# EBI-Metagenomics/deciphon-old

Measured on AMD Instinct MI355X. Metric: Gcell-updates/sec, higher is better.
Workload: dtype f32

## Files before the change

### deciphon-old_amd/__init__.py

```python
import ctypes as C
import os
import subprocess

import numpy as np

_HERE = os.path.dirname(os.path.abspath(__file__))
ROOT = os.path.dirname(_HERE)
LIB_PATH = os.path.join(_HERE, "libdcp_hip.so")
CSRC = os.path.join(_HERE, "csrc")

RC_OK, RC_END, RC_EFAIL, RC_EINVAL, RC_EIO, RC_ENOMEM, RC_EPARSE, RC_EAPI, RC_EHTTP = range(9)
RC_NAMES = ["RC_OK", "RC_END", "RC_EFAIL", "RC_EINVAL", "RC_EIO", "RC_ENOMEM", "RC_EPARSE",
            "RC_EAPI", "RC_EHTTP"]
ENTRY_DIST_NULL, ENTRY_DIST_UNIFORM, ENTRY_DIST_OCCUPANCY = 0, 1, 2
NCODES = 1364
NDIST = 129
NXTRANS = 13
CORE_SIZE_MAX = 4096
NUM_THREADS = 64

ABI_SYMBOLS = [
    "dcp_profile_new", "dcp_profile_sample", "dcp_profile_del", "dcp_profile_core_size",
    "dcp_profile_from_parts", "dcp_profile_entry_dist", "dcp_profile_epsilon", "dcp_rnd_seed", "dcp_rnd_next",
    "dcp_dist_unique_id", "dcp_dist_init", "dcp_dist_init_from_file", "dcp_dist_free", "dcp_dist_rank",
# ... 2 lines not shown
    "dcp_dist_comm_count", "dcp_dist_last_gather_ms", "dcp_plan_query_slots",
    "dcp_lprob_normalize", "dcp_h3reader_open_fp", "dcp_h3reader_next_params", "dcp_gpu_seqs_set_xtrans",
    "dcp_profile_accession", "dcp_profile_trans8", "dcp_profile_null_dist",
    "dcp_profile_insert_dist", "dcp_profile_match_dist", "dcp_frame_table_host", "dcp_xtrans",
    "dcp_lrt", "dcp_partition_by_count", "dcp_partition_by_cells", "dcp_gpu_device_count",
    "dcp_gpu_ctx_new", "dcp_gpu_ctx_del", "dcp_gpu_last_error", "dcp_gpu_stream",
    "dcp_gpu_db_upload", "dcp_gpu_db_nprofiles", "dcp_gpu_db_fetch_match_table",
    "dcp_gpu_db_one_layout", "dcp_gpu_db_table_bytes",
    "dcp_gpu_seqs_upload", "dcp_gpu_seqs_upload_text", "dcp_gpu_nseqs", "dcp_gpu_scan",
    "dcp_gpu_sync", "dcp_gpu_last_scan_kernel", "dcp_gpu_hit_buffer", "dcp_gpu_last_scan_redo_pairs", "dcp_gpu_last_scan_ms", "dcp_gpu_last_scan_launches", "dcp_gpu_fetch_scores",
    "dcp_gpu_fetch_hits", "dcp_gpu_scan_range", "dcp_gpu_set_hit_buffer",
    "dcp_gpu_last_scan_launch_info", "dcp_gpu_scan_cells", "dcp_gpu_scan_algorithmic_bytes",
    "dcp_gpu_trace_paths", "dcp_state_name", "dcp_profile_decode", "dcp_gc_decode",
    "dcp_prod_format_row", "dcp_prod_header", "dcp_h3reader_open", "dcp_h3reader_next",
    "dcp_h3reader_error", "dcp_h3reader_close", "dcp_swissprot_null_lprobs", "dcp_profile_consensus",
    "dcp_db_write", "dcp_db_open", "dcp_db_close", "dcp_db_nprofiles", "dcp_db_entry_dist", "dcp_db_epsilon",
    "dcp_db_profile_sizes", "dcp_db_partitions", "dcp_db_read",
    "dcp_profile_new64", "dcp_profile_sample64", "dcp_profile_precision", "dcp_profile_epsilon64",
    "dcp_profile_trans8_64", "dcp_profile_null_dist64", "dcp_profile_insert_dist64", "dcp_profile_match_dist64",
    "dcp_xtrans64", "dcp_gpu_db_upload64", "dcp_gpu_db_precision", "dcp_gpu_set_lrt_threshold64", "dcp_gpu_fetch_scores64", "dcp_gpu_fetch_hits64",
    "dcp_gpu_db_fetch_match_table64", "dcp_gpu_db_fetch_insert_null64", "dcp_gpu_trace_paths64",
    "dcp_gpu_seqs_set_xtrans64", "dcp_profile_from_parts64", "dcp_lprob_normalize64",
    "dcp_gpu_last_scan_query_plan",
]


class DcpError(RuntimeError):
    def __init__(self, rc, msg=""):
        self.rc = rc
        name = RC_NAMES[rc] if 0 <= rc < len(RC_NAMES) else str(rc)
        super().__init__(f"{name}: {msg}" if msg else name)


def build(verbose=False):
    subprocess.check_call(["make", "-C", CSRC] + ([] if verbose else ["-s"]))
    return LIB_PATH


class ScanParams(C.Structure):
    _fields_ = [("multi_hits", C.c_int), ("hmmer3_compat", C.c_int),
                ("lrt_threshold", C.c_float), ("keep_scores", C.c_int), ("kernel", C.c_int)]


KERNEL_AUTO, KERNEL_ROWSWEEP, KERNEL_QLANE, KERNEL_QLANE2 = 0, 1, 2, 3
KERNEL_QLANE64 = 4
DB_EXPAND_ON_HOST, DB_ONE_LAYOUT = 1, 2
# ... 45 lines not shown
        "dcp_partition_by_count": (U, [U, U, P]),
        "dcp_partition_by_cells": (None, [P, U, U, P]),
        "dcp_gpu_device_count": (I, []),
        "dcp_gpu_ctx_new": (P, [I]),
        "dcp_gpu_ctx_del": (None, [P]),
        "dcp_gpu_last_error": (C.c_char_p, [P]),
        "dcp_gpu_stream": (P, [P]),
        "dcp_gpu_db_upload": (I, [P, P, U, I]),
        "dcp_gpu_db_nprofiles": (U, [P]),
        "dcp_gpu_db_one_layout": (I, [P]),
        "dcp_gpu_db_table_bytes": (C.c_uint64, [P]),
        "dcp_gpu_db_fetch_match_table": (I, [P, U, P]),
        "dcp_gpu_seqs_upload": (I, [P, P, P, U]),
        "dcp_gpu_seqs_upload_text": (I, [P, C.c_char_p, P, U]),
        "dcp_gpu_nseqs": (U, [P]),
        "dcp_gpu_seqs_set_xtrans": (I, [P, P, U]),
        "dcp_gpu_scan": (I, [P, C.POINTER(ScanParams)]),
        "dcp_gpu_sync": (I, [P]),
        "dcp_gpu_last_scan_redo_pairs": (I, [P, C.POINTER(U)]),
        "dcp_gpu_last_scan_query_plan": (I, [P, C.POINTER(U), C.POINTER(C.c_ulonglong), C.POINTER(U), C.POINTER(U)]),
        "dcp_gpu_last_scan_ms": (F, [P]),
        "dcp_gpu_last_scan_launches": (U, [P]),
        "dcp_gpu_last_scan_kernel": (I, [P]),
        "dcp_gpu_fetch_scores": (I, [P, P, P]),
        "dcp_gpu_fetch_hits": (I, [P, P, U, C.POINTER(U)]),
        "dcp_gpu_scan_range": (I, [P, C.POINTER(ScanParams), U, U]),
        "dcp_gpu_set_hit_buffer": (I, [P, P, U, P]),
        "dcp_gpu_last_scan_launch_info": (I, [P, U, C.POINTER(LaunchInfo)]),
        "dcp_gpu_trace_paths": (I, [P, P, U, I, I, I, P, U, P, P]),
        "dcp_state_name": (U, [U, C.c_char_p]),
        "dcp_profile_decode": (I, [P, P, U, U, P]),
        "dcp_gc_decode": (C.c_char, [P]),
        "dcp_prod_format_row": (C.c_long, [C.c_char_p, C.c_size_t, C.c_int64, C.c_int64, C.c_char_p, C.c_char_p,
                                           C.c_double, C.c_double, C.c_char_p, C.c_char_p, P, P, U, P, U]),
        "dcp_prod_header": (C.c_char_p, []),
        "dcp_h3reader_open": (P, [C.c_char_p, I, F]),
        "dcp_h3reader_next": (I, [P, C.POINTER(P)]),
        "dcp_h3reader_error": (C.c_char_p, [P]),
        "dcp_h3reader_close": (None, [P]),
        "dcp_swissprot_null_lprobs": (None, [P]),
        "dcp_profile_consensus": (C.c_char_p, [P]),
        "dcp_db_write": (I, [C.c_char_p, P, U]),
        "dcp_db_open": (P, [C.c_char_p, C.POINTER(I)]),
        "dcp_db_close": (None, [P]),
        "dcp_db_nprofiles": (U, [P]),
        "dcp_db_entry_dist": (I, [P]),
# ... 483 lines not shown
        self._check(self._lib.dcp_gpu_test_set_trace_mode(self._c, int(bool(own_forward)), int(budget_floats)))

    def test_table_span(self, p):
        span, ldk, eb = C.c_uint(0), C.c_uint(0), C.c_uint(0)
        self._check(self._lib.dcp_gpu_test_fetch_table_span(self._c, p, None, 0, C.byref(span), C.byref(ldk),
                                                            C.byref(eb)))
        out = np.zeros((NCODES, span.value), np.float64 if eb.value == 8 else np.float32)
        self._check(self._lib.dcp_gpu_test_fetch_table_span(self._c, p, out.ctypes.data, out.nbytes, C.byref(span),
                                                            C.byref(ldk), C.byref(eb)))
        return out, ldk.value

    def test_set_rowsweep_variant(self, stage_rows, block_waves=0):
        self._check(self._lib.dcp_gpu_test_set_rowsweep_variant(self._c, int(stage_rows), int(block_waves)))

    @property
    def last_scan_ms(self):
        return self._lib.dcp_gpu_last_scan_ms(self._c)

    @property
    def last_scan_kernel(self):
        return self._lib.dcp_gpu_last_scan_kernel(self._c)

    @property
    def last_scan_launches(self):
        return self._lib.dcp_gpu_last_scan_launches(self._c)

    @property
    def last_scan_query_plan(self):
        nb, rows, prow, mg = C.c_uint(0), C.c_ulonglong(0), C.c_uint(0), C.c_uint(0)
        self._check(self._lib.dcp_gpu_last_scan_query_plan(self._c, C.byref(nb), C.byref(rows), C.byref(prow),
                                                           C.byref(mg)))
        return dict(nblocks=nb.value, sum_block_rows=rows.value, plane_rows=prow.value,
                    max_groups_per_slot=mg.value)

    @property
    def last_scan_redo_pairs(self):
        n = C.c_uint(0)
        self._check(self._lib.dcp_gpu_last_scan_redo_pairs(self._c, C.byref(n)))
        return n.value

    @property
    def cells(self):
        return self._lib.dcp_gpu_scan_cells(self._c)

    @property
    def algorithmic_bytes(self):
# ... 41 lines not shown
```

### deciphon-old_amd/csrc/dcp_gpu.hip

```cpp
#include "dcp_kernels.h"
#include "dcp_f64.h"

#include <hip/hip_runtime.h>

#include <algorithm>
#include <cmath>
#include <cstdarg>
#include <cstdio>
#include <cstring>
#include <limits>
#include <map>
#include <new>
#include <numeric>
#include <string>
#include <queue>
#include <type_traits>
#include <vector>

namespace
{

struct SizeClass
{
    int R, W;
// ... 139 lines not shown
    DevBuf<uint32_t> d_slot_first;
    unsigned ql_nqb = 0, ql_plane_rows = 0;
    unsigned ring_stall = 0;
    bool ring_check_pending = false;
    uint32_t *h_qstage = nullptr;
    size_t h_qstage_n = 0;
    hipEvent_t ev_qstage = nullptr;
    int rs_force_stg = -1;
    unsigned rs_force_bw = 0;
    unsigned rs_pad_lds = 0;
    int rs_force_pf = 0;
    int rs_force_R = 0;
    bool any_exact_e = false;
    DevBuf<unsigned> d_task_counter;
    DevBuf<dcp_pair> d_redo;
    DevBuf<unsigned> d_redo_n;
    bool redo_pending = false;
    unsigned last_redo_pairs = 0;
    struct dcp_scan_params last_prm = {};
    unsigned qorder_q0 = ~0u, qorder_q1 = ~0u, qorder_lmax = 0;
    unsigned num_cus = 0;
    int last_kernel = 0;
    unsigned qorder_nt = 0;
    int last_kernel_variant = 0;
    unsigned redo_cap_limit = 1u << 26;
    float last_ql_ms = 0;

    unsigned nseqs = 0;
    uint64_t total_len = 0;
    std::vector<uint32_t> seq_len;
    DevBuf<uint32_t> d_seq_words, d_seq_woff, d_seq_len;
    DevBuf<float> d_xtrans;
    int xt_multi = -1, xt_h3 = -1;
    bool xt_explicit = false;
    std::vector<double> xt64;

    ScanResults<float, dcp_hit> res;
    unsigned last_launches = 0;
    bool scanned = false;
    unsigned last_q0 = 0, last_q1 = 0;
    static constexpr int kMaxLaunches = 2 * kNumClasses + 1;
    hipEvent_t ev_class[kMaxLaunches] = {nullptr};
    hipStream_t class_stream[kNumClasses] = {nullptr};
    hipEvent_t ev_trace[kNumClasses + 1] = {nullptr};
    bool last_overlapped = false;
    int launched_class[kMaxLaunches] = {0};
// ... 1128 lines not shown
}

int dcp_gpu_hit_buffer(dcp_gpu_ctx *c, void **hits_dev, void **nhits_dev, unsigned *cap)
{
    if (!c || !hits_dev || !nhits_dev || !cap) return DCP_EINVAL;
    if (!c->scanned) return c->fail(DCP_EINVAL, "no scan yet");
    if (c->last_f64) return c->fail(DCP_EINVAL, "the last scan ran on a double DB: its hits are struct dcp_hit64 (dcp_gpu_fetch_hits64)");
    *hits_dev = c->res.hits();
    *nhits_dev = c->res.nhits();
    *cap = c->res.cap();
    return DCP_OK;
}

struct QlPlan
{
    std::vector<dcp_ql_group> groups;
    std::vector<uint32_t> slot_first;
    std::vector<uint32_t> block_rows;
    unsigned nqb = 0;
    unsigned plane_rows = 0;
    uint64_t sum_block_rows = 0;
    unsigned busy_slots = 0;
};
static QlPlan plan_query_groups(unsigned const *len_sorted, unsigned nq, unsigned slots)
{
    QlPlan pl;
    unsigned const ng = (nq + 63u) / 64u;
    struct G
    {
        unsigned first, n, lmax, rows;
    };
    std::vector<G> gs(ng);
    uint64_t sum_rows = 0;
    unsigned max_rows = 0;
    unsigned const rem = nq % 64u;
    for (unsigned g = 0; g < ng; ++g)
    {
        unsigned const first = rem == 0u ? g * 64u : (g == 0u ? 0u : rem + (g - 1u) * 64u);
        unsigned const n = rem != 0u && g == 0u ? rem : 64u;
        unsigned const lmax = len_sorted[first + n - 1u];
        gs[g] = G{first, n, lmax, dcp_qlane_group_rows(lmax)};
        sum_rows += gs[g].rows;
        max_rows = std::max(max_rows, gs[g].rows);
    }
    auto pack = [&](unsigned nqb, std::vector<std::vector<unsigned>> &slot_groups, std::vector<uint64_t> &load) {
        unsigned const S = nqb * slots;
        slot_groups.assign(S, {});
// ... 6 lines not shown
        {
            LS top = heap.top();
            heap.pop();
            slot_groups[top.second].push_back(g);
            load[top.second] += gs[g].rows;
            heap.push(LS(load[top.second], top.second));
        }
        std::vector<unsigned> order(S);
        for (unsigned i = 0; i < S; ++i)
            order[i] = i;
        std::stable_sort(order.begin(), order.end(), [&](unsigned x, unsigned y) { return load[x] > load[y]; });
        std::vector<std::vector<unsigned>> sg(S);
        std::vector<uint64_t> ld(S);
        for (unsigned i = 0; i < S; ++i)
            sg[i] = std::move(slot_groups[order[i]]), ld[i] = load[order[i]];
        slot_groups.swap(sg), load.swap(ld);
        uint64_t cost = 0;
        for (unsigned b = 0; b < nqb; ++b)
            cost += load[(size_t)b * slots];
        return cost;
    };
    unsigned const cap = (ng + slots - 1u) / slots;
    uint64_t const denom = (uint64_t)slots * max_rows;
    unsigned const lo = (unsigned)std::min<uint64_t>(std::max<uint64_t>(sum_rows / denom, 1), cap);
    unsigned const hi = (unsigned)std::min<uint64_t>(std::max<uint64_t>((sum_rows + denom - 1u) / denom, 1), cap);
    std::vector<std::vector<unsigned>> best_sg, sg;
    std::vector<uint64_t> best_ld, ld;
    uint64_t best_cost = ~0ull;
    unsigned best_nqb = 0;
    for (unsigned nqb = lo; nqb <= hi; ++nqb)
    {
        uint64_t const cost = pack(nqb, sg, ld);
        if (cost <= best_cost) best_cost = cost, best_nqb = nqb, best_sg.swap(sg), best_ld.swap(ld);
    }
    pl.nqb = best_nqb;
    pl.sum_block_rows = best_cost;
    pl.slot_first.assign((size_t)best_nqb * slots + 1u, 0);
    pl.block_rows.assign(best_nqb, 0);
    for (unsigned sidx = 0; sidx < best_nqb * slots; ++sidx)
    {
        pl.slot_first[sidx] = (uint32_t)pl.groups.size();
        uint32_t rowbase = 0;
        for (unsigned g : best_sg[sidx])
        {
            pl.groups.push_back(dcp_ql_group{gs[g].first, gs[g].n, rowbase, gs[g].lmax});
            rowbase += gs[g].rows;
        }
        pl.block_rows[sidx / slots] = std::max<uint32_t>(pl.block_rows[sidx / slots], rowbase);
        if (sidx < slots && rowbase) ++pl.busy_slots;
    }
    pl.slot_first.back() = (uint32_t)pl.groups.size();
    for (unsigned b = 0; b < best_nqb; ++b)
        pl.plane_rows = std::max(pl.plane_rows, pl.block_rows[b]);
    return pl;
}

namespace
{
struct SortedQueries
{
    std::vector<uint32_t> order;
    std::vector<unsigned> len;
    QlPlan plan;
};
}
static SortedQueries sorted_query_plan(dcp_gpu_ctx const *c, unsigned q_begin, unsigned q_end, unsigned slots)
{
    unsigned const nq = q_end - q_begin;
    SortedQueries s;
    s.order.resize(nq);
    std::iota(s.order.begin(), s.order.end(), 0u);
    std::stable_sort(s.order.begin(), s.order.end(),
                     [&](uint32_t x, uint32_t y) { return c->seq_len[q_begin + x] < c->seq_len[q_begin + y]; });
    s.len.resize(nq);
    for (unsigned i = 0; i < nq; ++i)
        s.len[i] = c->seq_len[q_begin + s.order[i]];
    s.plan = plan_query_groups(s.len.data(), nq, slots);
    return s;
}

extern "C" int dcp_plan_query_slots(unsigned const *len_sorted, unsigned nq, unsigned slots_per_block, unsigned *nblocks,
                                    unsigned long long *sum_block_rows, unsigned *plane_rows, unsigned *groups4,
                                    unsigned group_cap, unsigned *slot_first, unsigned slot_cap)
{
    if (!len_sorted || nq == 0 || (slots_per_block != 1u && slots_per_block != 4u) || !nblocks) return DCP_EINVAL;
    for (unsigned i = 1; i < nq; ++i)
        if (len_sorted[i] < len_sorted[i - 1]) return DCP_EINVAL;
    QlPlan const pl = plan_query_groups(len_sorted, nq, slots_per_block);
    *nblocks = pl.nqb;
    if (sum_block_rows) *sum_block_rows = pl.sum_block_rows;
    if (plane_rows) *plane_rows = pl.plane_rows;
    if (groups4)
    {
        if (group_cap < pl.groups.size()) return DCP_ENOMEM;
        std::memcpy(groups4, pl.groups.data(), pl.groups.size() * sizeof(dcp_ql_group));
    }
    if (slot_first)
    {
        if (slot_cap < pl.slot_first.size()) return DCP_ENOMEM;
        std::memcpy(slot_first, pl.slot_first.data(), pl.slot_first.size() * sizeof(uint32_t));
    }
    return DCP_OK;
}

static void rowsweep_variant(dcp_gpu_ctx const *c, int R, int W, unsigned nchunks, int *stg, unsigned *bw, int *pf)
{
    *pf = 0;
    if (W != 1)
    {
        *stg = 0, *bw = 1;
        return;
    }
    auto balanced = [&](unsigned maxw) {
        unsigned const nb = (nchunks + maxw - 1u) / maxw;
        return (nchunks + nb - 1u) / nb;
    };
    int g = 20;
    unsigned w = balanced(nchunks <= 56u ? 8u : 4u);
    unsigned const max84 = dcp_rowsweep_max_block_waves(R, W, 84);
    if (nchunks >= 6u && nchunks <= 36u && max84 != 0u)
    {
        unsigned const w84 = balanced(max84);
        unsigned const slots = dcp_rowsweep_max_block_waves(R, W, 84);
        unsigned const blocks = (160u * 1024u) / dcp_rowsweep_stage_bytes(R, 84);
        if (std::min(blocks * w84, slots) * 2u >= slots) g = 84, w = w84;
// ... 222 lines not shown
    double sum_len = 0;
    for (unsigned L : sorted.len)
        sum_len += L;
    unsigned const nqb = plan.nqb;
    double const sum_block_lmax = (double)plan.sum_block_rows;
    unsigned const lmax = sorted.len.back();
    double t_rs = (double)c->sum_core * (DCP_NCODES * 4.0) / 3e12 + qchunk * lmax * 1.2e-6;
    for (int k = 0; k < kNumClasses; ++k)
        t_rs += 1.05 * (double)c->class_core[k] * sum_len / kClassRate[k];
    unsigned const waves = std::max(1u, std::min(4u, plan.busy_slots));
    static double const kTrow[4] = {0.52, 0.54, 0.62, 0.73};
    double const trow = (w3 ? 0.56 : kTrow[waves - 1u]) * 1e-6;
    double const resident = (double)std::min<uint64_t>((uint64_t)c->nprof * nqb, (uint64_t)ql_blocks_per_cu * c->num_cus);
    double const t_ql = std::max((double)c->max_tiles * lmax * 0.52e-6,
                                 (double)c->sum_tiles * sum_block_lmax * trow / resident) +
                        1e-4;
    bool const stage2 = nq > 192u;
    double const fill = std::min(1.0, (double)c->nprof * nqb / (4.0 * c->num_cus));
    double const t_q = stage2 ? t_ql * (0.66 + 0.28 * fill) : t_ql;
    if (lmax > 200000u) return 1;
    return t_q < t_rs ? (stage2 ? 3 : 2) : 1;
}

static int ensure_qlane_layout(dcp_gpu_ctx *c, dcp_scan_args const &a, unsigned q_begin, unsigned q_end, unsigned ql_nt)
{
    if (!c->d_task_counter.p) HIP_TRY(c, c->d_task_counter.alloc(1));
    if (c->qorder_q0 == q_begin && c->qorder_q1 == q_end && c->qorder_nt == ql_nt) return DCP_OK;
    unsigned const nq = q_end - q_begin, NTq = ql_nt, slots = NTq / 64u;
    SortedQueries const sorted = sorted_query_plan(c, q_begin, q_end, slots);
    QlPlan const &plan = sorted.plan;
    unsigned const nqb = plan.nqb;
    if ((uint64_t)plan.plane_rows * NTq * 4u > 0xffffffffull)
        return c->fail(DCP_ENOMEM, "sequences too long for the query-lane kernel (%u plane rows): use kernel = 1", plan.plane_rows);
    size_t const nslot_words = (size_t)nqb * slots + 1u, ngroup_words = plan.groups.size() * 4u;
    size_t const need_stage = (size_t)nq + nqb + 1u + nslot_words + ngroup_words;
    if (!c->ev_qstage) HIP_TRY(c, hipEventCreateWithFlags(&c->ev_qstage, hipEventDisableTiming));
    else HIP_TRY(c, hipEventSynchronize(c->ev_qstage));
    if (c->h_qstage_n < need_stage)
    {
        if (c->h_qstage) (void)hipHostFree(c->h_qstage);
        c->h_qstage = nullptr, c->h_qstage_n = 0;
        HIP_TRY(c, hipHostMalloc((void **)&c->h_qstage, need_stage * sizeof(uint32_t), hipHostMallocDefault));
        c->h_qstage_n = need_stage;
    }
    uint32_t *const h_ord = c->h_qstage, *const wt_off = h_ord + nq, *const h_slots = wt_off + nqb + 1u,
                   *const h_groups = h_slots + nslot_words;
    static_assert(sizeof(dcp_ql_group) == 4 * sizeof(uint32_t), "group records travel as four words");
    std::memcpy(h_ord, sorted.order.data(), nq * sizeof(uint32_t));
    std::memcpy(h_slots, plan.slot_first.data(), nslot_words * sizeof(uint32_t));
    std::memcpy(h_groups, plan.groups.data(), ngroup_words * sizeof(uint32_t));
    uint64_t tot = 0;
    wt_off[0] = 0u;
    for (unsigned b = 0; b < nqb; ++b)
    {
        tot += ((uint64_t)plan.block_rows[b] + 8u) * NTq / 2u;
        if (tot > 0xffffffffull) return c->fail(DCP_EINVAL, "sequence batch too large");
        wt_off[b + 1u] = (uint32_t)tot;
    }
    if (c->d_qorder.n < nq) HIP_TRY(c, c->d_qorder.alloc(nq));
    if (c->d_wt_off.n < nqb + 1u) HIP_TRY(c, c->d_wt_off.alloc(nqb + 1u));
    if (c->d_slot_first.n < nslot_words) HIP_TRY(c, c->d_slot_first.alloc(nslot_words));
    if (c->d_ql_groups.n < plan.groups.size()) HIP_TRY(c, c->d_ql_groups.alloc(plan.groups.size()));
    if (c->d_words_t.n < tot) HIP_TRY(c, c->d_words_t.alloc((size_t)tot));
    HIP_TRY(c, hipMemcpyAsync(c->d_qorder.p, h_ord, nq * sizeof(uint32_t), hipMemcpyHostToDevice, c->stream));
    HIP_TRY(c, hipMemcpyAsync(c->d_wt_off.p, wt_off, (nqb + 1u) * sizeof(uint32_t), hipMemcpyHostToDevice, c->stream));
    HIP_TRY(c, hipMemcpyAsync(c->d_slot_first.p, h_slots, nslot_words * sizeof(uint32_t), hipMemcpyHostToDevice, c->stream));
    HIP_TRY(c, hipMemcpyAsync(c->d_ql_groups.p, h_groups, ngroup_words * sizeof(uint32_t), hipMemcpyHostToDevice, c->stream));
    HIP_TRY(c, hipEventRecord(c->ev_qstage, c->stream));
    dcp_qlane_args ta{};
    ta.seq_words = a.seq_words, ta.seq_woff = a.seq_woff, ta.seq_len = a.seq_len;
    ta.qorder = c->d_qorder.p, ta.words_t = c->d_words_t.p, ta.wt_off = c->d_wt_off.p;
    ta.groups = c->d_ql_groups.p, ta.slot_first = c->d_slot_first.p;
    ta.nseqs = nq, ta.nqblocks = nqb;
    if (dcp_launch_qlane_transpose(&ta, NTq, c->stream)) return c->fail(DCP_EFAIL, "no kernel for %u-query blocks", NTq);
    HIP_TRY(c, hipGetLastError());
    c->qorder_q0 = q_begin, c->qorder_q1 = q_end, c->qorder_nt = NTq;
    c->ql_nqb = nqb, c->ql_plane_rows = plan.plane_rows + 8u;
    return DCP_OK;
}

static int record_launch(dcp_gpu_ctx *c, int k, bool is_redo, hipStream_t stream, bool join)
{
    HIP_TRY(c, hipEventRecord(c->ev_class[c->n_launched], stream));
    if (join) HIP_TRY(c, hipStreamWaitEvent(c->stream, c->ev_class[c->n_launched], 0));
    c->launched_redo[c->n_launched] = is_redo;
    c->launched_class[c->n_launched++] = k;
    c->last_launches++;
    return DCP_OK;
}

static int launch_qlane_scan(dcp_gpu_ctx *c, struct dcp_scan_params const *prm, dcp_scan_args &a, unsigned NT,
                             unsigned ql_blocks_per_cu, bool two_stage, bool use_w3)
{
    dcp_qlane_args qa{};
    qa.profs = c->d_ql_metas.p;
    qa.emis_tiles = c->one_layout ? c->d_emis_match.p : c->d_emis_tiles.p;
    qa.tiles_from_rows = c->one_layout ? 1u : 0u;
    qa.emis_insert = c->d_emis_insert.p;
    qa.emis_null = c->d_emis_null.p;
    qa.ttrans = c->d_ttrans.p;
    qa.seq_words = a.seq_words;
    qa.seq_woff = a.seq_woff;
    qa.seq_len = a.seq_len;
// ... 28 lines not shown
        a.emis_match = c->d_emis_match.p;
        uint64_t tot = 0;
        uint64_t const cap_limit = c->redo_cap_limit;
        for (int k = 0; k < kNumClasses; ++k)
        {
            uint64_t const pairs = (uint64_t)a.nseqs * (c->class_first[k + 1] - c->class_first[k]);
            unsigned const cap = (unsigned)std::min<uint64_t>(pairs, cap_limit);
            qa.redo_base[k] = (unsigned)tot;
            qa.redo_cap[k] = cap;
            tot += cap;
            uint64_t const tpb = dcp_rowsweep_tasks_per_block(kClasses[k].W);
            uint64_t g = std::min<uint64_t>((cap + tpb - 1) / tpb, 8ull * c->num_cus);
            redo_grid[k] = (unsigned)((g + 7) / 8 * 8);
        }
        if (c->d_redo.n < tot) HIP_TRY(c, c->d_redo.alloc((size_t)tot));
    }
    if (!c->d_redo_n.p) HIP_TRY(c, c->d_redo_n.alloc(DCP_MAX_CLASSES + 2));
    HIP_TRY(c, hipMemsetAsync(c->d_redo_n.p, 0, (DCP_MAX_CLASSES + 2) * sizeof(unsigned), c->stream));
    qa.redo = c->d_redo.p;
    qa.redo_n = c->d_redo_n.p;
    qa.redo_overflow = c->d_redo_n.p + DCP_MAX_CLASSES;
    qa.ring_error = c->d_redo_n.p + DCP_MAX_CLASSES + 1;
    uint64_t const per_block = (uint64_t)dcp_qlane_scratch_planes() * (uint64_t)qa.plane_rows * NT;
    uint64_t const budget = (uint64_t)64 << 28;
    uint64_t fit = per_block ? budget / per_block : 0;
    uint64_t const resident_blocks = (uint64_t)ql_blocks_per_cu * c->num_cus;
    unsigned nblocks = (unsigned)std::min<uint64_t>(std::min<uint64_t>(ntasks, resident_blocks), fit);
    if (use_w3) nblocks = (nblocks + 2u) / 3u * 3u;
    if (nblocks == 0)
        return c->fail(DCP_ENOMEM, "sequences too long for the query-lane kernel (%u plane rows): use kernel = 1", qa.plane_rows);
    size_t const need = (size_t)nblocks * per_block;
    if (c->d_scratch.n < need) HIP_TRY(c, c->d_scratch.alloc(need));
    qa.scratch = c->d_scratch.p;
    HIP_TRY(c, hipMemsetAsync(c->d_task_counter.p, 0, sizeof(unsigned), c->stream));
    HIP_TRY(c, hipEventRecord(c->ev_start, c->stream));
    if (two_stage ? dcp_launch_qlane2(&qa, nblocks, c->stream)
                  : use_w3 ? dcp_launch_qlane_w3(&qa, nblocks / 3u, c->stream)
                           : dcp_launch_qlane(&qa, nblocks, NT, c->stream))
        return c->fail(DCP_EFAIL, "query-lane launch failed");
    HIP_TRY(c, hipGetLastError());
    if (int rc = record_launch(c, -1, false, c->stream, false)) return rc;
    for (int k = 0; redo && k < kNumClasses; ++k)
    {
        if (redo_grid[k] == 0) continue;
        a.pairs = c->d_redo.p + qa.redo_base[k];
        a.npairs = c->d_redo_n.p + k;
        a.pair_cap = qa.redo_cap[k];
        a.first_prof = 0;
        a.nprof = c->nprof;
        SizeClass const sc = kClasses[k];
        if (dcp_launch_rowsweep(sc.R, sc.W, &a, redo_grid[k], c->stream))
            return c->fail(DCP_EFAIL, "no kernel for class R=%d W=%d", sc.R, sc.W);
        if (int rc = record_launch(c, k, true, c->stream, false)) return rc;
    }
    HIP_TRY(c, hipGetLastError());
    HIP_TRY(c, hipEventRecord(c->ev_stop, c->stream));
    c->scanned = true;
    c->redo_pending = redo;
    c->ring_check_pending = two_stage;
    c->last_redo_pairs = 0;
    c->last_prm = *prm;
    return DCP_OK;
}

struct SegSweepPlan
{
    unsigned stride = 0;
    unsigned chunk[kNumClasses] = {0};
    uint64_t redo_off[kNumClasses] = {0}, col_rows = 0, redo_tot = 0;
};
static SegSweepPlan plan_segsweep(dcp_gpu_ctx const *c, unsigned q_begin, unsigned q_end)
{
    SegSweepPlan sp;
    unsigned const nq = q_end - q_begin;
    sp.stride = *std::max_element(c->seq_len.begin() + q_begin, c->seq_len.begin() + q_end) + 2u;
    for (int k = 0; k < kNumClasses; ++k)
// ... 149 lines not shown
        if (int rc = finish_scan(c)) return rc;
    if (!c->xt64.empty())
        return c->fail(DCP_EINVAL, "the explicit special transitions are double: a float DB takes them from dcp_gpu_seqs_set_xtrans");

    if (int rc = ensure_xtrans(c, prm->multi_hits, prm->hmmer3_compat)) return rc;
    HIP_TRY(c, c->res.ensure((size_t)c->nseqs * c->nprof, prm->keep_scores != 0));
    dcp_scan_args a = scan_args(c, prm, q_begin, q_end);
    unsigned const nq = q_end - q_begin;
    c->last_q0 = q_begin;
    c->last_q1 = q_end;

    unsigned ql_nt = dcp_qlane_block_size(), ql_blocks_per_cu = 2;
    bool const w3 = nq <= 64u;
    if (w3) ql_nt = 64u, ql_blocks_per_cu = 3;
    int kernel = prm->kernel;
    if (kernel == 0) kernel = choose_kernel(c, q_begin, q_end, a.qchunk, ql_nt, ql_blocks_per_cu, w3);
    if (kernel < 1 || kernel > 3) return c->fail(DCP_EINVAL, "unknown kernel %d", kernel);
    bool const two_stage = kernel == 3;
    c->last_kernel_variant = kernel;
    if (two_stage) kernel = 2;
    c->last_kernel = kernel;
    if (two_stage) ql_nt = dcp_qlane_block_size(), ql_blocks_per_cu = 1;
    if (kernel == 2)
        if (int rc = ensure_qlane_layout(c, a, q_begin, q_end, ql_nt)) return rc;

    HIP_TRY(c, hipMemsetAsync(a.nhits, 0, sizeof(unsigned), c->stream));
    c->last_launches = 0;
    c->n_launched = 0;
    if (kernel == 2) return launch_qlane_scan(c, prm, a, ql_nt, ql_blocks_per_cu, two_stage, w3 && !two_stage);
    return launch_rowsweep_scan(c, a, q_begin, q_end);
}

static int rerun_with_rowsweep(dcp_gpu_ctx *c)
{
    struct dcp_scan_params prm = c->last_prm;
    prm.kernel = 1;
    if (int rc = dcp_gpu_scan_range(c, &prm, c->last_q0, c->last_q1)) return rc;
    HIP_TRY(c, hipStreamSynchronize(c->stream));
    return DCP_OK;
}

static int finish_scan(dcp_gpu_ctx *c)
{
    HIP_TRY(c, hipStreamSynchronize(c->stream));
    if (c->f64.redo_pending)
    {
        c->f64.redo_pending = false;
// ... 17 lines not shown
        c->scanned = false;
        return c->fail(DCP_EFAIL, "query-lane kernel: the LDS ring hand-shake between the two stages timed out; the scan's results are invalid");
    }
    if (!redo) return DCP_OK;
    uint64_t tot = 0;
    for (int k = 0; k < kNumClasses; ++k)
        tot += n[k];
    c->last_redo_pairs = (unsigned)std::min<uint64_t>(tot, 0xffffffffull);
    if (n[DCP_MAX_CLASSES] == 0) return DCP_OK;
    return rerun_with_rowsweep(c);
}

#ifdef DCP_TEST_HOOKS
int dcp_gpu_test_set_rowsweep_variant(dcp_gpu_ctx *c, int stg, unsigned bw)
{
    if (!c) return DCP_EINVAL;
    c->rs_force_stg = stg;
    c->rs_force_bw = bw & 0xffu;
    c->rs_pad_lds = ((bw >> 8) & 0xffu) * 1024u;
    c->rs_force_pf = (int)((bw >> 16) & 1u);
    c->rs_force_R = (int)((bw >> 20) & 15u);
    c->seg_mode = ((bw >> 24) & 3u) == 1u ? 0 : ((bw >> 24) & 3u) == 2u ? 1 : -1;
    c->mp_mode = ((bw >> 26) & 3u) == 1u ? 0 : ((bw >> 26) & 3u) == 2u ? 1 : -1;
    return DCP_OK;
}
int dcp_gpu_test_set_seg_col_bytes(dcp_gpu_ctx *c, unsigned long long bytes)
{
    if (!c) return DCP_EINVAL;
    c->seg_col_bytes = bytes ? bytes : (uint64_t)6 << 30;
    return DCP_OK;
}
int dcp_gpu_test_set_ring_stall(dcp_gpu_ctx *c, int on)
{
    if (!c) return DCP_EINVAL;
    c->ring_stall = on ? 1u : 0u;
    return DCP_OK;
}
int dcp_gpu_test_set_trace_mode(dcp_gpu_ctx *c, int own_forward, unsigned long long budget_floats)
{
    if (!c) return DCP_EINVAL;
    c->trace_mode = own_forward ? 1 : 0;
    c->trace_budget = budget_floats;
    return DCP_OK;
}
int dcp_gpu_test_set_redo_cap(dcp_gpu_ctx *c, unsigned cap)
{
// ... 52 lines not shown
    if (!c->scanned) return c->fail(DCP_EINVAL, "no scan yet");
    HIP_TRY(c, hipSetDevice(c->device));
    if (int rc = finish_scan(c)) return rc;
    if (!c->last_f64 || c->last_kernel_variant != 4)
        return c->fail(DCP_EINVAL, "the last scan did not run the f64 query-lane kernel (kernel = 4): it has no batch plan");
    if (nblocks) *nblocks = c->f64.plan_blocks;
    if (sum_block_rows) *sum_block_rows = c->f64.plan_sum_rows;
    if (plane_rows) *plane_rows = c->f64.plan_rows;
    if (max_groups_per_slot) *max_groups_per_slot = c->f64.plan_max_groups;
    return DCP_OK;
}

float dcp_gpu_last_scan_ms(dcp_gpu_ctx *c)
{
    if (!c || !c->scanned) return -1.0f;
    float ms = -1.0f;
    if (hipEventSynchronize(c->ev_stop) != hipSuccess) return -1.0f;
    if (hipEventElapsedTime(&ms, c->ev_start, c->ev_stop) != hipSuccess) return -1.0f;
    return ms;
}

unsigned dcp_gpu_last_scan_launches(dcp_gpu_ctx const *c) { return c ? c->last_launches : 0; }
int dcp_gpu_last_scan_kernel(dcp_gpu_ctx const *c) { return c && c->scanned ? c->last_kernel_variant : 0; }

int dcp_gpu_last_scan_launch_info(dcp_gpu_ctx *c, unsigned i, struct dcp_launch_info *out)
{
    if (!c || !out || !c->scanned) return DCP_EINVAL;
    if (i >= c->n_launched) return DCP_EINVAL;
    int const k = c->launched_class[i];
    hipEvent_t const before = i == 0 || (c->last_kernel == 1 && c->last_overlapped) ? c->ev_start : c->ev_class[i - 1];
    if (hipEventSynchronize(c->ev_class[i]) != hipSuccess) return DCP_EFAIL;
    float ms = 0;
    if (hipEventElapsedTime(&ms, before, c->ev_class[i]) != hipSuccess) return DCP_EFAIL;
    out->ms = ms;
    if (k < 0)
    {
        out->nodes_per_lane = 4 * c->ql_G;
        out->waves_per_pair = 0;
        out->nprofiles = c->nprof;
        out->cells = dcp_gpu_scan_cells(c);
        out->algorithmic_bytes = dcp_gpu_scan_algorithmic_bytes(c);
        return DCP_OK;
    }
    uint64_t const np = c->class_first[k + 1] - c->class_first[k];
    out->nodes_per_lane = kClasses[k].R;
    out->waves_per_pair = kClasses[k].W;
    out->nprofiles = (unsigned)np;
    out->cells = out->algorithmic_bytes = 0;
    if (c->last_kernel == 2 || c->launched_redo[i]) return DCP_OK;
    uint64_t sumM = 0, len = 0;
    for (unsigned j = c->class_first[k]; j < c->class_first[k + 1]; ++j)
        sumM += c->metas[j].core_size;
    for (unsigned q = c->last_q0; q < c->last_q1; ++q)
// ... 307 lines not shown
```

### deciphon-old_amd/csrc/dcp_qlane.hip

```cpp
#include "dcp_kernels.h"

#include <hip/hip_runtime.h>
#include <type_traits>

namespace
{
constexpr int NC = DCP_NCODES;

#ifndef DCP_QLANE_RECOMPUTE_B
#define DCP_QLANE_RECOMPUTE_B 1
#endif
constexpr bool kRecomputeB = DCP_QLANE_RECOMPUTE_B != 0;
#ifndef DCP_QLANE_WD
#define DCP_QLANE_WD 5
#endif
constexpr unsigned kWD = DCP_QLANE_WD;
constexpr unsigned kPlanes = kRecomputeB ? 3u : 4u;
#ifndef DCP_QLANE_DIAG
#define DCP_QLANE_DIAG 0
#endif

#ifndef DCP_QL_WPLANE
#define DCP_QL_WPLANE 1
#endif
// ... 160 lines not shown
constexpr unsigned kL2Err = kL2Task + 8u;
constexpr unsigned kL2Tab1 = 65536u;
constexpr unsigned kL2Ring = 7u * kRingPlaneBytes;
constexpr unsigned kL2Bytes = kL2Ring + 3u * kRingPlaneBytes;
static_assert(kL2Task + 16u <= kL2Tab1 && kL2Tab1 + kL2TabIN <= kL2Ring && kL2Bytes == 160u * 1024u, "LDS layout");
static_assert((kL2Ring & (kRingPlaneBytes - 1u)) == 0u, "ring slots are addressed by OR");
static_assert(kRD >= 12u, "a shorter ring can deadlock the two stages (five-row hand-shake groups)");

__device__ __forceinline__ void compiler_fence() { asm volatile("" ::: "memory"); }
#define DCP_ISA_MARK(name) asm volatile("; " name ::: "memory")
__device__ __forceinline__ unsigned flag_load(lds_uint *flag)
{
    return __hip_atomic_load(flag, __ATOMIC_RELAXED, __HIP_MEMORY_SCOPE_WORKGROUP);
}
__device__ __forceinline__ void flag_store(lds_uint *flag, unsigned v)
{
    __hip_atomic_store(flag, v, __ATOMIC_RELAXED, __HIP_MEMORY_SCOPE_WORKGROUP);
}
#ifndef DCP_Q2_BOUND
#define DCP_Q2_BOUND 1
#endif
constexpr unsigned kRingSpinBound = 1u << 23;
constexpr unsigned kRingPoison = 0x7fffff00u;
__device__ __forceinline__ unsigned ring_wait(LdsLink const &lk, unsigned need)
{
    lds_uint *flag = (lds_uint *)(lk.base + lk.peer_flag);
    unsigned v = __builtin_amdgcn_readfirstlane(flag_load(flag));
#if DCP_Q2_BOUND
    unsigned spins = 0;
#pragma nounroll
    while (v < need)
    {
        __builtin_amdgcn_s_sleep(DCP_Q2_SLEEP);
        v = __builtin_amdgcn_readfirstlane(flag_load(flag));
        if (__builtin_expect(++spins == kRingSpinBound, 0))
        {
            typedef unsigned __attribute__((address_space(1))) *gerr_ptr;
            gerr_ptr const err = *(gerr_ptr __attribute__((address_space(3))) *)(lk.base + kL2Err);
            __hip_atomic_store(err, 1u, __ATOMIC_RELAXED, __HIP_MEMORY_SCOPE_AGENT);
            flag_store((lds_uint *)(lk.base + kL2Abort), 1u);
            flag_store(flag, kRingPoison);
            v = kRingPoison;
            __builtin_amdgcn_s_waitcnt(0x0070);
        }
    }
#else
// ... 633 lines not shown
        dcp_ql_prof const pm = a.profs[slot];
        unsigned const T = pm.ntiles;
        unsigned const sidx = __builtin_amdgcn_readfirstlane(qb * SLOTS + (tid >> 6));
        cu32 *sf = (cu32 *)(unsigned long long)a.slot_first;
        unsigned const g0 = sf[sidx], g1 = sf[sidx + 1u];
        uint32_t const *__restrict__ wordsT = a.words_t + __builtin_amdgcn_readfirstlane(a.wt_off[qb]);
        {
            float const *__restrict__ gi = a.emis_insert + (size_t)pm.pidx * NC;
            float const *__restrict__ gn = a.emis_null + (size_t)pm.pidx * NC;
            fill_tab_in<false>(lds + kL2TabIN / 4u, gi, gn, threadIdx.x, 512u);
        }
        bool const stalled = a.ring_stall != 0u && task == 0u && stage == 0u;

        unsigned const nsteps = (T + 1u) / 2u;
        unsigned const final_stage = (T - 1u) & 1u;
        GroupLane g;
        bool const single = g1 - g0 == 1u;
        bool t_loaded = false;
        for (unsigned st = 0; st < nsteps; ++st)
        {
            unsigned const t = 2u * st + stage;
            bool const mine = t < T;
            __syncthreads();
            if (mine) stage_tile_image<G, ROWS>(tabM, a, pm, t, tid, (unsigned)NT);
            flag_store((lds_uint *)(lk.base + lk.my_flag + tid * 4u), 0u);
            __syncthreads();
            if (!mine || (stalled && st == 0u) || __builtin_amdgcn_readfirstlane(*s_abort_p) != 0u) continue;
            cfloat *tt = as_const(a.ttrans + pm.ttrans_off + (size_t)t * (KT + 1) * 8);
            bool const first = t == 0u, last = t + 1u == T;
#if DCP_QLANE_DIAG & 4
#error "the two-stage kernel has no DIAG=4 build"
#endif
            for (unsigned gi = g0; gi < g1; ++gi)
            {
                if (!(single && t_loaded)) load_group(a, gi, tid & 63u, g);
                t_loaded = true;
                if (g.Lwave == 0u) continue;
                SweepOut o{ninf(), ninf(), ninf()};
                bool dirty = false;
#define QL2_SWEEP(F, L_, IN_, OUT_, TB_)                                                                  \
    ql_sweep<G, F, L_, NT, D, IN_, OUT_, TB_, false>(tt, lds, reinterpret_cast<float2 const *>(lds + (kL2TabIN - TB_ / 2u) / 4u), \
                                              wordsT, g.rowbase, g.L, g.Lwave, g.has, sc, plane, tid, g.xt, dirty, o, lk)
                if (stage == 0u)
                {
                    if (first && last) QL2_SWEEP(true, true, IO_HBM, IO_HBM, 0u);
                    else if (first) QL2_SWEEP(true, false, IO_HBM, IO_LDS, 0u);
                    else if (last) QL2_SWEEP(false, true, IO_HBM, IO_HBM, 0u);
// ... 195 lines not shown
```

### include/dcp_gpu.h

```cpp
#ifndef DCP_GPU_H
#define DCP_GPU_H

#include <stddef.h>
#include <stdint.h>
#include <stdio.h>

#ifdef __cplusplus
extern "C" {
#endif

enum dcp_rc
{
    DCP_OK = 0,
    DCP_END = 1,
    DCP_EFAIL = 2,
    DCP_EINVAL = 3,
    DCP_EIO = 4,
    DCP_ENOMEM = 5,
    DCP_EPARSE = 6,
    DCP_EAPI = 7,
    DCP_EHTTP = 8,
};

enum dcp_entry_dist
// ... 162 lines not shown

int dcp_gpu_scan(dcp_gpu_ctx *, struct dcp_scan_params const *);
int dcp_gpu_scan_range(dcp_gpu_ctx *, struct dcp_scan_params const *,
                       unsigned q_begin, unsigned q_end);
int dcp_gpu_set_hit_buffer(dcp_gpu_ctx *, void *hits_dev, unsigned cap,
                           void *nhits_dev);
int dcp_gpu_hit_buffer(dcp_gpu_ctx *, void **hits_dev, void **nhits_dev, unsigned *cap);
#ifdef DCP_TEST_HOOKS
int dcp_gpu_test_set_redo_cap(dcp_gpu_ctx *, unsigned cap);
int dcp_gpu_test_set_ring_stall(dcp_gpu_ctx *, int on);
int dcp_gpu_test_set_seg_col_bytes(dcp_gpu_ctx *, unsigned long long bytes);
int dcp_gpu_test_set_trace_mode(dcp_gpu_ctx *, int own_forward, unsigned long long budget_floats);
int dcp_gpu_test_set_rowsweep_variant(dcp_gpu_ctx *, int stage_rows, unsigned block_waves);
int dcp_gpu_test_fetch_table_span(dcp_gpu_ctx *, unsigned p, void *out, unsigned long long cap_bytes,
                                  unsigned *span, unsigned *ldk, unsigned *elem_bytes);
#endif
int dcp_gpu_sync(dcp_gpu_ctx *);
int dcp_gpu_last_scan_redo_pairs(dcp_gpu_ctx *, unsigned *npairs);
int dcp_gpu_last_scan_query_plan(dcp_gpu_ctx *, unsigned *nblocks, unsigned long long *sum_block_rows,
                                 unsigned *plane_rows, unsigned *max_groups_per_slot);
float dcp_gpu_last_scan_ms(dcp_gpu_ctx *);
unsigned dcp_gpu_last_scan_launches(dcp_gpu_ctx const *);
int dcp_gpu_last_scan_kernel(dcp_gpu_ctx const *);
struct dcp_launch_info
{
    int nodes_per_lane;
    int waves_per_pair;
    unsigned nprofiles;
    float ms;
    uint64_t cells;
    uint64_t algorithmic_bytes;
};
int dcp_gpu_last_scan_launch_info(dcp_gpu_ctx *, unsigned i,
                                  struct dcp_launch_info *out);

int dcp_gpu_fetch_scores(dcp_gpu_ctx *, float *null_out, float *alt_out);
int dcp_gpu_fetch_hits(dcp_gpu_ctx *, struct dcp_hit *hits, unsigned cap,
                       unsigned *nhits);
int dcp_gpu_fetch_scores64(dcp_gpu_ctx *, double *null_out, double *alt_out);
int dcp_gpu_fetch_hits64(dcp_gpu_ctx *, struct dcp_hit64 *hits, unsigned cap, unsigned *nhits);
struct dcp_step
{
    uint16_t state_id;
    uint8_t seqlen;
    uint8_t reserved;
};
// ... 31 lines not shown
void dcp_dist_free(dcp_dist *);
int dcp_dist_rank(dcp_dist const *);
int dcp_dist_nranks(dcp_dist const *);
int dcp_dist_comm_count(dcp_dist const *);
double dcp_dist_last_gather_ms(dcp_dist const *);
char const *dcp_dist_last_error(dcp_dist const *);
void dcp_dist_shard(unsigned const *core_sizes, unsigned nprofiles, int nranks, int rank, unsigned *begin,
                    unsigned *end);
int dcp_dist_gather_scan_hits(dcp_dist *, dcp_gpu_ctx *ctx, unsigned profile_offset, int root,
                              struct dcp_hit **out, unsigned *nout);
int dcp_dist_gather_hits(dcp_dist *, void const *hits_dev, void const *nhits_dev, unsigned cap,
                         unsigned profile_offset, int root, void *scan_stream, struct dcp_hit **out,
                         unsigned *nout);
int dcp_dist_gather_plan(uint32_t const *meta, int nranks, unsigned *counts, unsigned *profile_offset,
                         uint64_t *displ, int *any_overflow, int *any_failed, uint64_t *total);
void dcp_dist_free_hits(struct dcp_hit *hits);
long dcp_dist_merge_hits(unsigned const *counts, unsigned const *profile_offset, int nranks,
                         struct dcp_hit const *records, struct dcp_hit *out, unsigned cap);

int dcp_plan_query_slots(unsigned const *len_sorted, unsigned nq, unsigned slots_per_block, unsigned *nblocks,
                         unsigned long long *sum_block_rows, unsigned *plane_rows, unsigned *groups4,
                         unsigned group_cap, unsigned *slot_first, unsigned slot_cap);

uint64_t dcp_gpu_scan_cells(dcp_gpu_ctx const *);
uint64_t dcp_gpu_scan_algorithmic_bytes(dcp_gpu_ctx const *);

#ifdef __cplusplus
}
#endif
#endif
```

Before: 1423.

## Merge query blocks in the query-lane plan and fork redo launches onto class streams

The query-lane planner may now merge up to four query blocks into fewer, taller blocks. It does so only when enough tasks remain to fill the resident blocks, total block rows do not grow, and the scratch budget still fits. Fewer query blocks mean each profile table is streamed fewer times across query blocks. Redo rowsweep launches now run on per-class streams after the query-lane kernel, in reverse class order, so they overlap each other instead of running serially. The risks are lower parallelism or load balance from merged blocks and more stream synchronisation overhead.

```diff
diff --git a/deciphon-old_amd/__init__.py b/deciphon-old_amd/__init__.py
--- a/deciphon-old_amd/__init__.py
+++ b/deciphon-old_amd/__init__.py
@@ -48,6 +48,7 @@
     "dcp_gpu_db_fetch_match_table64", "dcp_gpu_db_fetch_insert_null64", "dcp_gpu_trace_paths64",
     "dcp_gpu_seqs_set_xtrans64", "dcp_profile_from_parts64", "dcp_lprob_normalize64",
     "dcp_gpu_last_scan_query_plan",
+    "dcp_plan_query_slots_for_scan", "dcp_qlane_max_merge", "dcp_gpu_last_scan_query_blocks",
 ]
 
 
@@ -139,6 +140,7 @@
         "dcp_gpu_last_scan_ms": (F, [P]),
         "dcp_gpu_last_scan_launches": (U, [P]),
         "dcp_gpu_last_scan_kernel": (I, [P]),
+        "dcp_gpu_last_scan_query_blocks": (U, [P]),
         "dcp_gpu_fetch_scores": (I, [P, P, P]),
         "dcp_gpu_fetch_hits": (I, [P, P, U, C.POINTER(U)]),
         "dcp_gpu_scan_range": (I, [P, C.POINTER(ScanParams), U, U]),
@@ -668,6 +670,10 @@
         return self._lib.dcp_gpu_last_scan_kernel(self._c)
 
     @property
+    def last_scan_query_blocks(self):
+        return self._lib.dcp_gpu_last_scan_query_blocks(self._c)
+
+    @property
     def last_scan_launches(self):
         return self._lib.dcp_gpu_last_scan_launches(self._c)
 
diff --git a/deciphon-old_amd/csrc/dcp_gpu.hip b/deciphon-old_amd/csrc/dcp_gpu.hip
--- a/deciphon-old_amd/csrc/dcp_gpu.hip
+++ b/deciphon-old_amd/csrc/dcp_gpu.hip
@@ -185,6 +185,8 @@
     unsigned num_cus = 0;
     int last_kernel = 0;
     unsigned qorder_nt = 0;
+    unsigned qorder_merge = 0;
+    unsigned ql_merge_force = 0;
     int last_kernel_variant = 0;
     unsigned redo_cap_limit = 1u << 26;
     float last_ql_ms = 0;
@@ -1359,7 +1361,7 @@
     uint64_t sum_block_rows = 0;
     unsigned busy_slots = 0;
 };
-static QlPlan plan_query_groups(unsigned const *len_sorted, unsigned nq, unsigned slots)
+static QlPlan plan_query_groups(unsigned const *len_sorted, unsigned nq, unsigned slots, unsigned max_blocks = 0)
 {
     QlPlan pl;
     unsigned const ng = (nq + 63u) / 64u;
@@ -1412,8 +1414,9 @@
     };
     unsigned const cap = (ng + slots - 1u) / slots;
     uint64_t const denom = (uint64_t)slots * max_rows;
-    unsigned const lo = (unsigned)std::min<uint64_t>(std::max<uint64_t>(sum_rows / denom, 1), cap);
-    unsigned const hi = (unsigned)std::min<uint64_t>(std::max<uint64_t>((sum_rows + denom - 1u) / denom, 1), cap);
+    unsigned lo = (unsigned)std::min<uint64_t>(std::max<uint64_t>(sum_rows / denom, 1), cap);
+    unsigned hi = (unsigned)std::min<uint64_t>(std::max<uint64_t>((sum_rows + denom - 1u) / denom, 1), cap);
+    if (max_blocks) lo = std::min(lo, max_blocks), hi = std::min(hi, max_blocks);
     std::vector<std::vector<unsigned>> best_sg, sg;
     std::vector<uint64_t> best_ld, ld;
     uint64_t best_cost = ~0ull;
@@ -1445,6 +1448,33 @@
     return pl;
 }
 
+constexpr uint64_t kQlScratchBudget = (uint64_t)64 << 28;
+#ifndef DCP_QL_MAX_MERGE
+#define DCP_QL_MAX_MERGE 4
+#endif
+constexpr unsigned kQlMaxMerge = DCP_QL_MAX_MERGE;
+static QlPlan plan_query_groups_for_scan(unsigned const *len_sorted, unsigned nq, unsigned slots, unsigned nprof,
+                                         unsigned resident_blocks, unsigned max_merge)
+{
+    QlPlan const full = plan_query_groups(len_sorted, nq, slots);
+    if (max_merge <= 1u || full.nqb <= 1u) return full;
+    uint64_t const floor_tasks = 8ull * resident_blocks;
+    uint64_t const by_tasks = nprof ? (floor_tasks + nprof - 1u) / nprof : ~0ull;
+    uint64_t const by_merge = ((uint64_t)full.nqb + max_merge - 1u) / max_merge;
+    uint64_t const lanes = (uint64_t)slots * 64u;
+    for (uint64_t nb = std::max<uint64_t>(std::max(by_tasks, by_merge), 1); nb < full.nqb; ++nb)
+    {
+        QlPlan pl = plan_query_groups(len_sorted, nq, slots, (unsigned)nb);
+        if ((uint64_t)nprof * pl.nqb < floor_tasks || ((uint64_t)full.nqb + pl.nqb - 1u) / pl.nqb > max_merge) continue;
+        if (pl.sum_block_rows > full.sum_block_rows) continue;
+        uint64_t const rows = (uint64_t)pl.plane_rows + 8u;
+        if (rows * lanes * 4u > 0xffffffffull) continue;
+        if (std::max<uint64_t>(resident_blocks, 1) * dcp_qlane_scratch_planes() * rows * lanes > kQlScratchBudget) continue;
+        return pl;
+    }
+    return full;
+}
+
 namespace
 {
 struct SortedQueries
@@ -1454,7 +1484,8 @@
     QlPlan plan;
 };
 }
-static SortedQueries sorted_query_plan(dcp_gpu_ctx const *c, unsigned q_begin, unsigned q_end, unsigned slots)
+static SortedQueries sorted_query_plan(dcp_gpu_ctx const *c, unsigned q_begin, unsigned q_end, unsigned slots,
+                                       unsigned resident_blocks = 0, unsigned max_merge = 0)
 {
     unsigned const nq = q_end - q_begin;
     SortedQueries s;
@@ -1465,18 +1496,14 @@
     s.len.resize(nq);
     for (unsigned i = 0; i < nq; ++i)
         s.len[i] = c->seq_len[q_begin + s.order[i]];
-    s.plan = plan_query_groups(s.len.data(), nq, slots);
+    s.plan = max_merge ? plan_query_groups_for_scan(s.len.data(), nq, slots, c->nprof, resident_blocks, max_merge)
+                       : plan_query_groups(s.len.data(), nq, slots);
     return s;
 }
 
-extern "C" int dcp_plan_query_slots(unsigned const *len_sorted, unsigned nq, unsigned slots_per_block, unsigned *nblocks,
-                                    unsigned long long *sum_block_rows, unsigned *plane_rows, unsigned *groups4,
-                                    unsigned group_cap, unsigned *slot_first, unsigned slot_cap)
-{
-    if (!len_sorted || nq == 0 || (slots_per_block != 1u && slots_per_block != 4u) || !nblocks) return DCP_EINVAL;
-    for (unsigned i = 1; i < nq; ++i)
-        if (len_sorted[i] < len_sorted[i - 1]) return DCP_EINVAL;
-    QlPlan const pl = plan_query_groups(len_sorted, nq, slots_per_block);
+static int plan_out(QlPlan const &pl, unsigned *nblocks, unsigned long long *sum_block_rows, unsigned *plane_rows,
+                    unsigned *groups4, unsigned group_cap, unsigned *slot_first, unsigned slot_cap)
+{
     *nblocks = pl.nqb;
     if (sum_block_rows) *sum_block_rows = pl.sum_block_rows;
     if (plane_rows) *plane_rows = pl.plane_rows;
@@ -1491,6 +1518,35 @@
         std::memcpy(slot_first, pl.slot_first.data(), pl.slot_first.size() * sizeof(uint32_t));
     }
     return DCP_OK;
+}
+static bool ascending(unsigned const *len_sorted, unsigned nq)
+{
+    for (unsigned i = 1; i < nq; ++i)
+        if (len_sorted[i] < len_sorted[i - 1]) return false;
+    return true;
+}
+
+extern "C" int dcp_plan_query_slots(unsigned const *len_sorted, unsigned nq, unsigned slots_per_block, unsigned *nblocks,
+                                    unsigned long long *sum_block_rows, unsigned *plane_rows, unsigned *groups4,
+                                    unsigned group_cap, unsigned *slot_first, unsigned slot_cap)
+{
+    if (!len_sorted || nq == 0 || (slots_per_block != 1u && slots_per_block != 4u) || !nblocks) return DCP_EINVAL;
+    if (!ascending(len_sorted, nq)) return DCP_EINVAL;
+    return plan_out(plan_query_groups(len_sorted, nq, slots_per_block), nblocks, sum_block_rows, plane_rows, groups4,
+                    group_cap, slot_first, slot_cap);
+}
+
+extern "C" unsigned dcp_qlane_max_merge(void) { return kQlMaxMerge; }
+
+extern "C" int dcp_plan_query_slots_for_scan(unsigned const *len_sorted, unsigned nq, unsigned slots_per_block,
+                                             unsigned nprof, unsigned resident_blocks, unsigned max_merge,
+                                             unsigned *nblocks, unsigned long long *sum_block_rows, unsigned *plane_rows,
+                                             unsigned *groups4, unsigned group_cap, unsigned *slot_first, unsigned slot_cap)
+{
+    if (!len_sorted || nq == 0 || (slots_per_block != 1u && slots_per_block != 4u) || !nblocks || nprof == 0) return DCP_EINVAL;
+    if (!ascending(len_sorted, nq)) return DCP_EINVAL;
+    return plan_out(plan_query_groups_for_scan(len_sorted, nq, slots_per_block, nprof, resident_blocks, max_merge), nblocks,
+                    sum_block_rows, plane_rows, groups4, group_cap, slot_first, slot_cap);
 }
 
 static void rowsweep_variant(dcp_gpu_ctx const *c, int R, int W, unsigned nchunks, int *stg, unsigned *bw, int *pf)
@@ -1759,12 +1815,17 @@
     return t_q < t_rs ? (stage2 ? 3 : 2) : 1;
 }
 
-static int ensure_qlane_layout(dcp_gpu_ctx *c, dcp_scan_args const &a, unsigned q_begin, unsigned q_end, unsigned ql_nt)
+static int ensure_qlane_layout(dcp_gpu_ctx *c, dcp_scan_args const &a, unsigned q_begin, unsigned q_end, unsigned ql_nt,
+                               unsigned ql_blocks_per_cu)
 {
     if (!c->d_task_counter.p) HIP_TRY(c, c->d_task_counter.alloc(1));
-    if (c->qorder_q0 == q_begin && c->qorder_q1 == q_end && c->qorder_nt == ql_nt) return DCP_OK;
+    unsigned const max_merge = ql_nt != dcp_qlane_block_size() ? 0u : c->ql_merge_force ? c->ql_merge_force : kQlMaxMerge;
+    unsigned const resident_blocks = c->ql_merge_force ? 0u : ql_blocks_per_cu * c->num_cus;
+    unsigned const merge_key = max_merge << 16 | (max_merge ? (c->ql_merge_force ? 0xffffu : ql_blocks_per_cu) : 0u);
+    if (c->qorder_q0 == q_begin && c->qorder_q1 == q_end && c->qorder_nt == ql_nt && c->qorder_merge == merge_key) return DCP_OK;
+    c->qorder_q0 = c->qorder_q1 = ~0u;
     unsigned const nq = q_end - q_begin, NTq = ql_nt, slots = NTq / 64u;
-    SortedQueries const sorted = sorted_query_plan(c, q_begin, q_end, slots);
+    SortedQueries const sorted = sorted_query_plan(c, q_begin, q_end, slots, resident_blocks, max_merge);
     QlPlan const &plan = sorted.plan;
     unsigned const nqb = plan.nqb;
     if ((uint64_t)plan.plane_rows * NTq * 4u > 0xffffffffull)
@@ -1811,11 +1872,14 @@
     ta.nseqs = nq, ta.nqblocks = nqb;
     if (dcp_launch_qlane_transpose(&ta, NTq, c->stream)) return c->fail(DCP_EFAIL, "no kernel for %u-query blocks", NTq);
     HIP_TRY(c, hipGetLastError());
-    c->qorder_q0 = q_begin, c->qorder_q1 = q_end, c->qorder_nt = NTq;
+    c->qorder_q0 = q_begin, c->qorder_q1 = q_end, c->qorder_nt = NTq, c->qorder_merge = merge_key;
     c->ql_nqb = nqb, c->ql_plane_rows = plan.plane_rows + 8u;
     return DCP_OK;
 }
 
+#ifndef DCP_QL_FORK_REDO
+#define DCP_QL_FORK_REDO 1
+#endif
 static int record_launch(dcp_gpu_ctx *c, int k, bool is_redo, hipStream_t stream, bool join)
 {
     HIP_TRY(c, hipEventRecord(c->ev_class[c->n_launched], stream));
@@ -1890,7 +1954,7 @@
     qa.redo_overflow = c->d_redo_n.p + DCP_MAX_CLASSES;
     qa.ring_error = c->d_redo_n.p + DCP_MAX_CLASSES + 1;
     uint64_t const per_block = (uint64_t)dcp_qlane_scratch_planes() * (uint64_t)qa.plane_rows * NT;
-    uint64_t const budget = (uint64_t)64 << 28;
+    uint64_t const budget = kQlScratchBudget;
     uint64_t fit = per_block ? budget / per_block : 0;
     uint64_t const resident_blocks = (uint64_t)ql_blocks_per_cu * c->num_cus;
     unsigned nblocks = (unsigned)std::min<uint64_t>(std::min<uint64_t>(ntasks, resident_blocks), fit);
@@ -1908,18 +1972,24 @@
         return c->fail(DCP_EFAIL, "query-lane launch failed");
     HIP_TRY(c, hipGetLastError());
     if (int rc = record_launch(c, -1, false, c->stream, false)) return rc;
-    for (int k = 0; redo && k < kNumClasses; ++k)
-    {
+    bool const fork = redo && DCP_QL_FORK_REDO != 0;
+    c->last_overlapped = fork;
+    hipEvent_t const ev_ql = c->ev_class[c->n_launched - 1u];
+    for (int kk = 0; redo && kk < kNumClasses; ++kk)
+    {
+        int const k = fork ? kNumClasses - 1 - kk : kk;
         if (redo_grid[k] == 0) continue;
+        hipStream_t const ls = fork ? c->class_stream[k] : c->stream;
+        if (fork) HIP_TRY(c, hipStreamWaitEvent(ls, ev_ql, 0));
         a.pairs = c->d_redo.p + qa.redo_base[k];
         a.npairs = c->d_redo_n.p + k;
         a.pair_cap = qa.redo_cap[k];
         a.first_prof = 0;
         a.nprof = c->nprof;
         SizeClass const sc = kClasses[k];
-        if (dcp_launch_rowsweep(sc.R, sc.W, &a, redo_grid[k], c->stream))
+        if (dcp_launch_rowsweep(sc.R, sc.W, &a, redo_grid[k], ls))
             return c->fail(DCP_EFAIL, "no kernel for class R=%d W=%d", sc.R, sc.W);
-        if (int rc = record_launch(c, k, true, c->stream, false)) return rc;
+        if (int rc = record_launch(c, k, true, ls, fork)) return rc;
     }
     HIP_TRY(c, hipGetLastError());
     HIP_TRY(c, hipEventRecord(c->ev_stop, c->stream));
@@ -2115,7 +2185,7 @@
     c->last_kernel = kernel;
     if (two_stage) ql_nt = dcp_qlane_block_size(), ql_blocks_per_cu = 1;
     if (kernel == 2)
-        if (int rc = ensure_qlane_layout(c, a, q_begin, q_end, ql_nt)) return rc;
+        if (int rc = ensure_qlane_layout(c, a, q_begin, q_end, ql_nt, ql_blocks_per_cu)) return rc;
 
     HIP_TRY(c, hipMemsetAsync(a.nhits, 0, sizeof(unsigned), c->stream));
     c->last_launches = 0;
@@ -2179,6 +2249,7 @@
     c->rs_force_R = (int)((bw >> 20) & 15u);
     c->seg_mode = ((bw >> 24) & 3u) == 1u ? 0 : ((bw >> 24) & 3u) == 2u ? 1 : -1;
     c->mp_mode = ((bw >> 26) & 3u) == 1u ? 0 : ((bw >> 26) & 3u) == 2u ? 1 : -1;
+    c->ql_merge_force = (bw >> 28) & 15u;
     return DCP_OK;
 }
 int dcp_gpu_test_set_seg_col_bytes(dcp_gpu_ctx *c, unsigned long long bytes)
@@ -2277,13 +2348,19 @@
 
 unsigned dcp_gpu_last_scan_launches(dcp_gpu_ctx const *c) { return c ? c->last_launches : 0; }
 int dcp_gpu_last_scan_kernel(dcp_gpu_ctx const *c) { return c && c->scanned ? c->last_kernel_variant : 0; }
+unsigned dcp_gpu_last_scan_query_blocks(dcp_gpu_ctx const *c)
+{
+    return c && c->scanned && !c->last_f64 && c->last_kernel == 2 ? c->ql_nqb : 0u;
+}
 
 int dcp_gpu_last_scan_launch_info(dcp_gpu_ctx *c, unsigned i, struct dcp_launch_info *out)
 {
     if (!c || !out || !c->scanned) return DCP_EINVAL;
     if (i >= c->n_launched) return DCP_EINVAL;
     int const k = c->launched_class[i];
-    hipEvent_t const before = i == 0 || (c->last_kernel == 1 && c->last_overlapped) ? c->ev_start : c->ev_class[i - 1];
+    hipEvent_t const before = i == 0 || (c->last_kernel == 1 && c->last_overlapped) ? c->ev_start
+                              : c->last_kernel == 2 && c->last_overlapped           ? c->ev_class[0]
+                                                                                    : c->ev_class[i - 1];
     if (hipEventSynchronize(c->ev_class[i]) != hipSuccess) return DCP_EFAIL;
     float ms = 0;
     if (hipEventElapsedTime(&ms, before, c->ev_class[i]) != hipSuccess) return DCP_EFAIL;
diff --git a/deciphon-old_amd/csrc/dcp_qlane.hip b/deciphon-old_amd/csrc/dcp_qlane.hip
--- a/deciphon-old_amd/csrc/dcp_qlane.hip
+++ b/deciphon-old_amd/csrc/dcp_qlane.hip
@@ -206,6 +206,7 @@
 #endif
 constexpr unsigned kRingSpinBound = 1u << 23;
 constexpr unsigned kRingPoison = 0x7fffff00u;
+static_assert(kRingPoison > (0xffffffffu / (kRLanes * 4u)) + 16u, "the poison must be a row no sweep reaches");
 __device__ __forceinline__ unsigned ring_wait(LdsLink const &lk, unsigned need)
 {
     lds_uint *flag = (lds_uint *)(lk.base + lk.peer_flag);
@@ -885,7 +886,7 @@
             unsigned const t = 2u * st + stage;
             bool const mine = t < T;
             __syncthreads();
-            if (mine) stage_tile_image<G, ROWS>(tabM, a, pm, t, tid, (unsigned)NT);
+            if (mine && !((DCP_QLANE_DIAG & 16) != 0 && st > 0u)) stage_tile_image<G, ROWS>(tabM, a, pm, t, tid, (unsigned)NT);
             flag_store((lds_uint *)(lk.base + lk.my_flag + tid * 4u), 0u);
             __syncthreads();
             if (!mine || (stalled && st == 0u) || __builtin_amdgcn_readfirstlane(*s_abort_p) != 0u) continue;
diff --git a/include/dcp_gpu.h b/include/dcp_gpu.h
--- a/include/dcp_gpu.h
+++ b/include/dcp_gpu.h
@@ -208,6 +208,7 @@
 float dcp_gpu_last_scan_ms(dcp_gpu_ctx *);
 unsigned dcp_gpu_last_scan_launches(dcp_gpu_ctx const *);
 int dcp_gpu_last_scan_kernel(dcp_gpu_ctx const *);
+unsigned dcp_gpu_last_scan_query_blocks(dcp_gpu_ctx const *);
 struct dcp_launch_info
 {
     int nodes_per_lane;
@@ -285,6 +286,12 @@
                          unsigned long long *sum_block_rows, unsigned *plane_rows, unsigned *groups4,
                          unsigned group_cap, unsigned *slot_first, unsigned slot_cap);
 
+int dcp_plan_query_slots_for_scan(unsigned const *len_sorted, unsigned nq, unsigned slots_per_block, unsigned nprof,
+                                  unsigned resident_blocks, unsigned max_merge, unsigned *nblocks,
+                                  unsigned long long *sum_block_rows, unsigned *plane_rows, unsigned *groups4,
+                                  unsigned group_cap, unsigned *slot_first, unsigned slot_cap);
+unsigned dcp_qlane_max_merge(void);
+
 uint64_t dcp_gpu_scan_cells(dcp_gpu_ctx const *);
 uint64_t dcp_gpu_scan_algorithmic_bytes(dcp_gpu_ctx const *);
 
```

After: 1430, median of 6. About the same (+0.5%).
